# lab-emi/CleanUMamba

Measured on AMD Instinct MI355X. Metric: audio samples/sec/node (train step, E8, 10s@16kHz), higher is better.
Workload: dtype f16

## Files before the change

cleanumamba_amd/csrc/fft_lds.h:

```cpp
#pragma once
#include "common.h"

namespace cum {

__device__ __forceinline__ float2 cmul(float2 a, float2 b) { return make_float2(a.x * b.x - a.y * b.y, a.x * b.y + a.y * b.x); }
__device__ __forceinline__ float2 conjf2(float2 a) { return make_float2(a.x, -a.y); }
__device__ __forceinline__ float2 packed_bin(float2 za, float2 zb, float2 w) {
  const float2 c1 = make_float2(0.5f * (1.f + w.y), -0.5f * w.x), c2 = make_float2(0.5f * (1.f - w.y), 0.5f * w.x);
  const float2 p = cmul(c1, za), q = cmul(c2, conjf2(zb));
  return make_float2(p.x + q.x, p.y + q.y);
}
__device__ __forceinline__ double2 cmul(double2 a, double2 b) { return make_double2(a.x * b.x - a.y * b.y, a.x * b.y + a.y * b.x); }
__device__ __forceinline__ double2 packed_bin(double2 za, double2 zb, double2 w) {
  const double2 c1 = make_double2(0.5 * (1.0 + w.y), -0.5 * w.x), c2 = make_double2(0.5 * (1.0 - w.y), 0.5 * w.x);
  const double2 p = cmul(c1, za), q = cmul(c2, make_double2(zb.x, -zb.y));
  return make_double2(p.x + q.x, p.y + q.y);
}

template <typename T>
struct FftVec;
template <>
struct FftVec<float> {
  typedef float4 v4;
  typedef float2 v2;
  __device__ static __forceinline__ float4 mk4(float a, float b, float c, float d) { return make_float4(a, b, c, d); }
  __device__ static __forceinline__ float2 mk2(float a, float b) { return make_float2(a, b); }
};
template <>
struct FftVec<double> {
  typedef double4 v4;
  typedef double2 v2;
  __device__ static __forceinline__ double4 mk4(double a, double b, double c, double d) { return make_double4(a, b, c, d); }
  __device__ static __forceinline__ double2 mk2(double a, double b) { return make_double2(a, b); }
};

template <int H, typename T = float>
struct FusedFft {
  typedef typename FftVec<T>::v4 V4;
  typedef typename FftVec<T>::v2 V2;
  __device__ static __forceinline__ V4 mk4(T a, T b, T c, T d) { return FftVec<T>::mk4(a, b, c, d); }
  __device__ static __forceinline__ V2 mk2(T a, T b) { return FftVec<T>::mk2(a, b); }
  static constexpr int LOGH = H == 256 ? 8 : H == 512 ? 9 : 10;
  static constexpr bool LEAD2 = (LOGH & 1) != 0;
  static constexpr int PER = H / 64;
  static constexpr int SLOTS = H + H / 16;
  static constexpr int UNR = H == 1024 ? 2 : 1;

  __device__ static __forceinline__ int pad(int e) { return e + (e >> 4); }

  __device__ static __forceinline__ int pos(int k) {
    int p = 0, rem = k, L = H;
    if constexpr (LEAD2) {
      p = (rem & 1) * (H / 2);
      rem >>= 1;
      L = H / 2;
    }
#pragma unroll
    for (int s = 0; s < (LOGH / 2); ++s) {
      p += (rem & 3) * (L >> 2);
      rem >>= 2;
      L >>= 2;
    }
    return p;
  }

  __device__ static __forceinline__ V2 twiddle(const V2 *tw, int e, int L) {
    int m = e * (2 * H / L);
    const bool neg = m > H;
    m = neg ? m - H : m;
    V2 w = tw[m];
    if (neg) { w.x = -w.x; w.y = -w.y; }
    return w;
  }

  __device__ static __forceinline__ V4 cmul4(V4 v, V2 w) {
    return mk4(v.x * w.x - v.y * w.y, v.x * w.y + v.y * w.x, v.z * w.x - v.w * w.y, v.z * w.y + v.w * w.x);
  }
  __device__ static __forceinline__ V4 add4(V4 a, V4 b) { return mk4(a.x + b.x, a.y + b.y, a.z + b.z, a.w + b.w); }
  __device__ static __forceinline__ V4 sub4(V4 a, V4 b) { return mk4(a.x - b.x, a.y - b.y, a.z - b.z, a.w - b.w); }

  __device__ static __forceinline__ void stage_fence() {
    __builtin_amdgcn_fence(__ATOMIC_RELEASE, "wavefront");
    __builtin_amdgcn_wave_barrier();
    __builtin_amdgcn_fence(__ATOMIC_ACQUIRE, "wavefront");
  }

  __device__ static __forceinline__ void forward(V4 *buf, const V2 *tw, int lane) {
    int L = H;
    if constexpr (LEAD2) {
#pragma unroll UNR
      for (int i = 0; i < H / 128; ++i) {
        const int j = lane + 64 * i;
        const V4 a = buf[pad(j)], b = buf[pad(j + H / 2)];
        buf[pad(j)] = add4(a, b);
        buf[pad(j + H / 2)] = cmul4(sub4(a, b), twiddle(tw, j, H));
      }
      L = H / 2;
      stage_fence();
    }
#pragma unroll
    for (int st = 0; st < LOGH / 2; ++st, L >>= 2) {
      const int q4 = L >> 2;
#pragma unroll UNR
      for (int i = 0; i < H / 256; ++i) {
        const int q = lane + 64 * i;
        const int j = q & (q4 - 1), p = ((q - j) << 2) + j;
        const V4 a = buf[pad(p)], b = buf[pad(p + q4)], c = buf[pad(p + 2 * q4)], d = buf[pad(p + 3 * q4)];
        const V4 t0 = add4(a, c), t1 = sub4(a, c), t2 = add4(b, d), u = sub4(b, d);
        const V4 t3 = mk4(u.y, -u.x, u.w, -u.z);
        buf[pad(p)] = add4(t0, t2);
        if (L > 4) {
          buf[pad(p + q4)] = cmul4(add4(t1, t3), twiddle(tw, j, L));
          buf[pad(p + 2 * q4)] = cmul4(sub4(t0, t2), twiddle(tw, 2 * j, L));
          buf[pad(p + 3 * q4)] = cmul4(sub4(t1, t3), twiddle(tw, 3 * j, L));
        } else {
          buf[pad(p + q4)] = add4(t1, t3);
          buf[pad(p + 2 * q4)] = sub4(t0, t2);
          buf[pad(p + 3 * q4)] = sub4(t1, t3);
        }
      }
      stage_fence();
    }
  }

  __device__ static __forceinline__ void inverse_xy(V4 *buf, const V2 *tw, int lane) {
    auto ld = [&](int e) { const V4 v = buf[pad(e)]; return mk2(v.x, v.y); };
    auto st2 = [&](int e, float2 v) { float2 *q = reinterpret_cast<float2 *>(&buf[pad(e)]); *q = v; };
    auto cmulc = [](float2 v, float2 w) { return make_float2(v.x * w.x + v.y * w.y, v.y * w.x - v.x * w.y); };
    int L = 4;
#pragma unroll
    for (int stg = 0; stg < LOGH / 2; ++stg, L <<= 2) {
      const int q4 = L >> 2;
#pragma unroll UNR
      for (int i = 0; i < H / 256; ++i) {
        const int q = lane + 64 * i;
        const int j = q & (q4 - 1), p = ((q - j) << 2) + j;
        float2 a = ld(p), b = ld(p + q4), c = ld(p + 2 * q4), d = ld(p + 3 * q4);
        if (L > 4) {
          b = cmulc(b, twiddle(tw, j, L));
          c = cmulc(c, twiddle(tw, 2 * j, L));
          d = cmulc(d, twiddle(tw, 3 * j, L));
        }
        const float2 s0 = make_float2(a.x + c.x, a.y + c.y), s1 = make_float2(a.x - c.x, a.y - c.y);
        const float2 s2 = make_float2(b.x + d.x, b.y + d.y), u = make_float2(b.x - d.x, b.y - d.y);
        const float2 s3 = make_float2(-u.y, u.x);
        st2(p, make_float2(s0.x + s2.x, s0.y + s2.y));
        st2(p + q4, make_float2(s1.x + s3.x, s1.y + s3.y));
        st2(p + 2 * q4, make_float2(s0.x - s2.x, s0.y - s2.y));
        st2(p + 3 * q4, make_float2(s1.x - s3.x, s1.y - s3.y));
      }
      stage_fence();
    }
    if constexpr (LEAD2) {
#pragma unroll UNR
      for (int i = 0; i < H / 128; ++i) {
        const int j = lane + 64 * i;
        const float2 a = ld(j), b = cmulc(ld(j + H / 2), twiddle(tw, j, H));
        st2(j, make_float2(a.x + b.x, a.y + b.y));
        st2(j + H / 2, make_float2(a.x - b.x, a.y - b.y));
      }
      stage_fence();
    }
  }
};

}
```

cleanumamba_amd/csrc/stft_loss.hip:

```cpp
#include "common.h"
#include "fft_lds.h"

namespace cum {

constexpr int kLossRows = 8;
constexpr float kClamp = 1e-7f;

__device__ __forceinline__ int64_t reflect_index(int64_t s, int64_t len) {
  if (s < 0) s = -s;
  if (s >= len) s = 2 * (len - 1) - s;
  return s;
}

__global__ __launch_bounds__(256) void stft_frames_kernel(const float *__restrict__ x, int64_t len, int64_t x_sb,
                                                          int n_fft, int hop, int win_len,
                                                          const float *__restrict__ window,
                                                          float *__restrict__ frames, int64_t n_frames) {
  const int64_t f = blockIdx.x, b = blockIdx.y;
  const int off = (n_fft - win_len) / 2;
  const float *xb = x + b * x_sb;
  float *dst = frames + (b * n_frames + f) * n_fft;
  const int64_t s0 = f * hop - n_fft / 2;
  for (int n4 = threadIdx.x * 4; n4 < n_fft; n4 += 256 * 4) {
    float v[4];
// ... 112 lines not shown
          dm *= inv_mx * ((k == 0 || k == bins - 1) ? 1.f : 0.5f);
          out = make_float2(dm * vx.x, dm * vx.y);
        }
      }
      z[base + k] = out;
    }
  }
}

__global__ __launch_bounds__(256) void stft_loss_partials_packed_kernel(const float2 *__restrict__ zx,
                                                                        const float2 *__restrict__ zy, int64_t rows,
                                                                        int64_t n_frames, int H, int64_t frame0,
                                                                        const float2 *__restrict__ tw,
                                                                        float *__restrict__ partials) {
  __shared__ float red[4];
  const int64_t r0 = (int64_t)blockIdx.x * kLossRows;
  const int nrow = (int)min((int64_t)kLossRows, rows - r0);
  float s1 = 0.f, s2 = 0.f, s3 = 0.f;
  for (int r = 0; r < nrow; ++r) {
    if ((r0 + r) % n_frames < frame0) continue;
    const int64_t base = (r0 + r) * H;
    for (int k = threadIdx.x; k <= H; k += 256) {
      const int a = k == H ? 0 : k, b = k == 0 ? 0 : H - k;
      const float2 w = tw[k];
      const LossTerms t = loss_terms(packed_bin(zx[base + a], zx[base + b], w), packed_bin(zy[base + a], zy[base + b], w));
      const float d = t.my - t.mx;
      s1 += d * d;
      s2 += t.my * t.my;
      s3 += fabsf(logf(t.my) - logf(t.mx));
    }
  }
  s1 = block_sum_256(s1, red);
  s2 = block_sum_256(s2, red);
  s3 = block_sum_256(s3, red);
  if (threadIdx.x == 0) {
    partials[3 * (int64_t)blockIdx.x + 0] = s1;
    partials[3 * (int64_t)blockIdx.x + 1] = s2;
    partials[3 * (int64_t)blockIdx.x + 2] = s3;
  }
}

__device__ __forceinline__ float2 bin_grad(float2 vx, float2 vy, float c_sc, float c_mag) {
  const LossTerms t = loss_terms(vx, vy);
  if (!t.live) return make_float2(0.f, 0.f);
  const float inv_mx = 1.f / t.mx;
  const float lg = logf(t.mx) - logf(t.my);
  const float sgn = lg > 0.f ? 1.f : (lg < 0.f ? -1.f : 0.f);
  const float dm = (c_sc * (t.mx - t.my) + c_mag * sgn * inv_mx) * inv_mx;
  return make_float2(dm * vx.x, dm * vx.y);
}

__global__ __launch_bounds__(256) void stft_loss_grad_packed_kernel(const float2 *__restrict__ zx,
                                                                    const float2 *__restrict__ zy, int64_t rows,
                                                                    int64_t n_frames, int H, int64_t frame0,
                                                                    const float *__restrict__ stats,
                                                                    const float *__restrict__ g_sc,
                                                                    const float *__restrict__ g_mag, float inv_count,
                                                                    const float2 *__restrict__ tw,
                                                                    float2 *__restrict__ gz) {
  const int64_t r0 = (int64_t)blockIdx.x * kLossRows;
  const int nrow = (int)min((int64_t)kLossRows, rows - r0);
  const float c_sc = g_sc[0] / (stats[2] * stats[3]);
  const float c_mag = g_mag[0] * inv_count;
  for (int r = 0; r < nrow; ++r) {
    const bool in_band = (r0 + r) % n_frames >= frame0;
    const int64_t base = (r0 + r) * H;
    for (int j = threadIdx.x; j <= H / 2; j += 256) {
      const int m = j == 0 ? 0 : H - j;
      float2 oj = make_float2(0.f, 0.f), om = oj;
      if (in_band) {
        const float2 xj = zx[base + j], xm = zx[base + m], yj = zy[base + j], ym = zy[base + m];
        if (j == 0) {
          const float2 g0 = bin_grad(make_float2(xj.x + xj.y, 0.f), make_float2(yj.x + yj.y, 0.f), c_sc, c_mag);
          const float2 gh = bin_grad(make_float2(xj.x - xj.y, 0.f), make_float2(yj.x - yj.y, 0.f), c_sc, c_mag);
          oj = make_float2(g0.x + gh.x, g0.x - gh.x);
        } else {
          const float2 wj = tw[j], wm = tw[H - j];
          const float2 gj = bin_grad(packed_bin(xj, xm, wj), packed_bin(yj, ym, wj), c_sc, c_mag);
          const float2 gm = bin_grad(packed_bin(xm, xj, wm), packed_bin(ym, yj, wm), c_sc, c_mag);
          const float2 c1j = make_float2(0.5f * (1.f + wj.y), 0.5f * wj.x), c2j = make_float2(0.5f * (1.f - wj.y), 0.5f * wj.x);
          const float2 c1m = make_float2(0.5f * (1.f + wm.y), 0.5f * wm.x), c2m = make_float2(0.5f * (1.f - wm.y), 0.5f * wm.x);
          const float2 a = cmul(c1j, gj), b = cmul(c2m, conjf2(gm));
          oj = make_float2(a.x + b.x, a.y + b.y);
          const float2 c = cmul(c1m, gm), d = cmul(c2j, conjf2(gj));
          om = make_float2(c.x + d.x, c.y + d.y);
        }
      }
      gz[base + j] = oj;
      if (m != j) gz[base + m] = om;
    }
  }
}

__global__ __launch_bounds__(256) void stft_fold_kernel(const float *__restrict__ dframes, int64_t len, int n_fft,
                                                        int hop, int win_len, const float *__restrict__ window,
                                                        int64_t n_frames, float *__restrict__ dx, int64_t dx_sb,
                                                        int accumulate) {
  const int64_t m = (int64_t)blockIdx.x * 256 + threadIdx.x, b = blockIdx.y;
  if (m >= len) return;
  const int off = (n_fft - win_len) / 2, half = n_fft / 2;
  const float *src = dframes + b * n_frames * n_fft;
  float acc = 0.f;
  int64_t pos[3];
  int npos = 0;
  pos[npos++] = m + half;
  if (m >= 1 && m <= half) pos[npos++] = half - m;
  if (m <= len - 2 && m >= len - 1 - half) pos[npos++] = half + 2 * (len - 1) - m;
  for (int i = 0; i < npos; ++i) {
    const int64_t p = pos[i];
    if (p - off < 0) continue;
    int64_t f_hi = (p - off) / hop;
    if (f_hi > n_frames - 1) f_hi = n_frames - 1;
    int64_t f_lo = p - off - win_len + 1;
    f_lo = f_lo <= 0 ? 0 : (f_lo + hop - 1) / hop;
    for (int64_t f = f_lo; f <= f_hi; ++f) {
      const int n = (int)(p - f * hop);
      acc += window[n - off] * src[f * n_fft + n];
    }
  }
  float *o = dx + b * dx_sb + m;
  *o = accumulate ? *o + acc : acc;
}


__device__ __forceinline__ void fused_terms(float2 sx, float2 sy, float &s1, float &s2, float &s3) {
  const float px = fmaxf(sx.x * sx.x + sx.y * sx.y, kClamp), py = fmaxf(sy.x * sy.x + sy.y * sy.y, kClamp);
  const float d = __builtin_amdgcn_sqrtf(py) - __builtin_amdgcn_sqrtf(px);
  s1 = fmaf(d, d, s1);
  s2 += py;
  s3 += (0.5f * kLn2) * fabsf(__builtin_amdgcn_logf(py) - __builtin_amdgcn_logf(px));
}

__device__ __forceinline__ float2 fused_bin_grad(float2 vx, float2 vy, float c_sc, float c_mag) {
  const float pxr = vx.x * vx.x + vx.y * vx.y;
  if (!(pxr >= kClamp)) return make_float2(0.f, 0.f);
  const float py = fmaxf(vy.x * vy.x + vy.y * vy.y, kClamp);
  const float inv_mx = __builtin_amdgcn_rsqf(pxr);
  const float mx = pxr * inv_mx, my = __builtin_amdgcn_sqrtf(py);
  const float sgn = pxr > py ? 1.f : (pxr < py ? -1.f : 0.f);
  const float dm = (c_sc * (mx - my) + c_mag * sgn * inv_mx) * inv_mx;
  return make_float2(dm * vx.x, dm * vx.y);
}

struct FusedStftParams {
  const float *x, *y, *window, *tw;
  int64_t len, x_sb, y_sb, n_frames, frame0, n_total;
  int hop, win_len;
  float *partials;
  const float *stats, *g_sc, *g_mag;
  float inv_count;
  float *dframes;
};

template <int H>
__device__ __forceinline__ void fused_load_frame(const FusedStftParams &p, int64_t b, int64_t f, int lane, float4 *buf) {
  typedef FusedFft<H> F;
  const int n_fft = 2 * H, off = (n_fft - p.win_len) / 2;
  const float *xb = p.x + b * p.x_sb, *yb = p.y + b * p.y_sb;
  const int64_t s0 = f * p.hop - H;
  const bool inner = s0 >= 0 && s0 + n_fft <= p.len && ((off | p.win_len) & 1) == 0 &&
                     ((((uintptr_t)(xb + s0)) | ((uintptr_t)(yb + s0)) | ((uintptr_t)p.window)) & 7) == 0;
#pragma unroll 2
  for (int i = 0; i < F::PER; ++i) {
    const int m = lane + 64 * i, n = 2 * m;
    float4 z = make_float4(0.f, 0.f, 0.f, 0.f);
    if (n + 1 >= off && n < off + p.win_len) {
      float x0, x1, y0, y1, w0, w1;
      if (inner) {
        const float2 xv = *reinterpret_cast<const float2 *>(xb + s0 + n), yv = *reinterpret_cast<const float2 *>(yb + s0 + n);
        const float2 wv = *reinterpret_cast<const float2 *>(p.window + (n - off));
        x0 = xv.x; x1 = xv.y; y0 = yv.x; y1 = yv.y; w0 = wv.x; w1 = wv.y;
      } else {
        const int64_t i0 = reflect_index(s0 + n, p.len), i1 = reflect_index(s0 + n + 1, p.len);
        x0 = xb[i0]; x1 = xb[i1]; y0 = yb[i0]; y1 = yb[i1];
        const int wi = n - off;
        w0 = (wi >= 0 && wi < p.win_len) ? p.window[wi] : 0.f;
        w1 = (wi + 1 >= 0 && wi + 1 < p.win_len) ? p.window[wi + 1] : 0.f;
      }
      z = make_float4(w0 * x0, w1 * x1, w0 * y0, w1 * y1);
    }
    buf[F::pad(m)] = z;
  }
}

template <int H>
__device__ __forceinline__ void fused_load_tables(const FusedStftParams &p, float2 *tw) {
  for (int k = threadIdx.x; k <= H; k += blockDim.x) tw[k] = reinterpret_cast<const float2 *>(p.tw)[k];
  __syncthreads();
}

constexpr int kFusedWaves = 4;

template <int H>
__global__ __launch_bounds__(64 * kFusedWaves) __attribute__((amdgpu_waves_per_eu(H == 256 ? 6 : (H == 512 ? 4 : 2)))) void stft_fused_fwd_kernel(const FusedStftParams p) {
  typedef FusedFft<H> F;
  __shared__ __attribute__((aligned(16))) float4 s_buf[kFusedWaves][F::SLOTS];
  __shared__ float2 s_tw[H + 1];
  __shared__ float s_red[3][kFusedWaves];
  const int lane = threadIdx.x & 63, wave = uniform(threadIdx.x >> 6);
  fused_load_tables<H>(p, s_tw);
  float4 *buf = s_buf[wave];
  float s1 = 0.f, s2 = 0.f, s3 = 0.f;
  const int nw = gridDim.x * kFusedWaves, n_total = (int)p.n_total, n_frames = (int)p.n_frames;
  for (int fr = blockIdx.x * kFusedWaves + wave; fr < n_total; fr += nw) {
    const int b = fr / n_frames, f = fr - b * n_frames;
    if (f < p.frame0) continue;
    fused_load_frame<H>(p, b, f, lane, buf);
    F::stage_fence();
    F::forward(buf, s_tw, lane);
#pragma unroll 1
    for (int i = 0; i <= F::PER / 2; ++i) {
      const int j = lane + 64 * i;
      if (j > H / 2) break;
      const int m = j == 0 ? 0 : H - j;
      const float4 vj = buf[F::pad(F::pos(j))], vm = buf[F::pad(F::pos(m))];
      const float2 xj = make_float2(vj.x, vj.y), yj = make_float2(vj.z, vj.w), xm = make_float2(vm.x, vm.y), ym = make_float2(vm.z, vm.w);
      if (j == 0) {
        fused_terms(make_float2(xj.x + xj.y, 0.f), make_float2(yj.x + yj.y, 0.f), s1, s2, s3);
        fused_terms(make_float2(xj.x - xj.y, 0.f), make_float2(yj.x - yj.y, 0.f), s1, s2, s3);
      } else {
        const float2 wj = s_tw[j];
        fused_terms(packed_bin(xj, xm, wj), packed_bin(yj, ym, wj), s1, s2, s3);
        if (m != j) {
          const float2 wm = s_tw[m];
          fused_terms(packed_bin(xm, xj, wm), packed_bin(ym, yj, wm), s1, s2, s3);
        }
      }
    }
    F::stage_fence();
  }
  float v[3] = {s1, s2, s3};
#pragma unroll
  for (int j = 0; j < 3; ++j) {
#pragma unroll
    for (int o = 32; o >= 1; o >>= 1) v[j] += __shfl_xor(v[j], o, 64);
    if (lane == 0) s_red[j][wave] = v[j];
  }
  __syncthreads();
  if (threadIdx.x < 3) {
    float t = 0.f;
#pragma unroll
    for (int w = 0; w < kFusedWaves; ++w) t += s_red[threadIdx.x][w];
    p.partials[3 * (int64_t)blockIdx.x + threadIdx.x] = t;
  }
}

template <int H>
__global__ __launch_bounds__(64 * kFusedWaves) __attribute__((amdgpu_waves_per_eu(H == 256 ? 6 : (H == 512 ? 4 : 2)))) void stft_fused_bwd_kernel(const FusedStftParams p) {
  typedef FusedFft<H> F;
  __shared__ __attribute__((aligned(16))) float4 s_buf[kFusedWaves][F::SLOTS];
  __shared__ float2 s_tw[H + 1];
  const int lane = threadIdx.x & 63, wave = uniform(threadIdx.x >> 6);
  fused_load_tables<H>(p, s_tw);
  float4 *buf = s_buf[wave];
  const float c_sc = p.g_sc[0] / (p.stats[2] * p.stats[3]);
  const float c_mag = p.g_mag[0] * p.inv_count;
  const int n_fft = 2 * H, off = (n_fft - p.win_len) / 2;
  const int nw = gridDim.x * kFusedWaves, n_total = (int)p.n_total, n_frames = (int)p.n_frames;
  for (int fr = blockIdx.x * kFusedWaves + wave; fr < n_total; fr += nw) {
    const int b = fr / n_frames, f = fr - b * n_frames;
    float *dst = p.dframes + (int64_t)fr * n_fft;
    if (f < p.frame0) {
#pragma unroll
      for (int i = 0; i < F::PER; ++i) {
        const int n = 2 * (lane + 64 * i);
        if (n + 1 >= off && n < off + p.win_len) *reinterpret_cast<float2 *>(dst + n) = make_float2(0.f, 0.f);
      }
      continue;
    }
    fused_load_frame<H>(p, b, f, lane, buf);
    F::stage_fence();
    F::forward(buf, s_tw, lane);
#pragma unroll 1
    for (int i = 0; i <= F::PER / 2; ++i) {
      const int j = lane + 64 * i;
      if (j > H / 2) break;
      const int m = j == 0 ? 0 : H - j;
      const int pj = F::pad(F::pos(j)), pm = F::pad(F::pos(m));
      const float4 vj = buf[pj], vm = buf[pm];
      const float2 xj = make_float2(vj.x, vj.y), yj = make_float2(vj.z, vj.w), xm = make_float2(vm.x, vm.y), ym = make_float2(vm.z, vm.w);
      float2 oj, om = make_float2(0.f, 0.f);
      if (j == 0) {
        const float2 g0 = fused_bin_grad(make_float2(xj.x + xj.y, 0.f), make_float2(yj.x + yj.y, 0.f), c_sc, c_mag);
        const float2 gh = fused_bin_grad(make_float2(xj.x - xj.y, 0.f), make_float2(yj.x - yj.y, 0.f), c_sc, c_mag);
        oj = make_float2(g0.x + gh.x, g0.x - gh.x);
      } else {
        const float2 wj = s_tw[j], wm = s_tw[H - j];
        const float2 gj = fused_bin_grad(packed_bin(xj, xm, wj), packed_bin(yj, ym, wj), c_sc, c_mag);
        const float2 gm = fused_bin_grad(packed_bin(xm, xj, wm), packed_bin(ym, yj, wm), c_sc, c_mag);
        const float2 c1j = make_float2(0.5f * (1.f + wj.y), 0.5f * wj.x), c2j = make_float2(0.5f * (1.f - wj.y), 0.5f * wj.x);
        const float2 c1m = make_float2(0.5f * (1.f + wm.y), 0.5f * wm.x), c2m = make_float2(0.5f * (1.f - wm.y), 0.5f * wm.x);
        const float2 a = cmul(c1j, gj), bq = cmul(c2m, conjf2(gm));
        oj = make_float2(a.x + bq.x, a.y + bq.y);
        const float2 c = cmul(c1m, gm), d = cmul(c2j, conjf2(gj));
        om = make_float2(c.x + d.x, c.y + d.y);
      }
      *reinterpret_cast<float2 *>(&buf[pj]) = oj;
      if (m != j) *reinterpret_cast<float2 *>(&buf[pm]) = om;
    }
    F::stage_fence();
    F::inverse_xy(buf, s_tw, lane);
#pragma unroll
    for (int i = 0; i < F::PER; ++i) {
      const int mm = lane + 64 * i, n = 2 * mm;
      if (n + 1 >= off && n < off + p.win_len) {
        const float4 v = buf[F::pad(mm)];
        *reinterpret_cast<float2 *>(dst + n) = make_float2(v.x, v.y);
      }
    }
    F::stage_fence();
  }
}

}

using namespace cum;

static int check_resolution(int64_t len, int n_fft, int hop, int win_len, int64_t n_frames) {
  CUM_REQUIRE(n_fft >= 8 && n_fft % 4 == 0 && hop > 0 && win_len > 0 && win_len <= n_fft, "stft: bad resolution");
  CUM_REQUIRE(len > n_fft / 2, "stft: signal shorter than the reflect padding");
  CUM_REQUIRE(n_frames == 1 + len / hop, "stft: n_frames must be 1 + len / hop");
  return CUM_OK;
}

extern "C" int cum_stft_frames(const float *x, int64_t batch, int64_t len, int64_t x_stride_b, int32_t n_fft,
                               int32_t hop, int32_t win_length, const float *window, float *frames, int64_t n_frames,
                               void *stream) {
  CUM_REQUIRE(batch >= 0 && batch < 65536, "stft_frames: bad batch");
  if (int rc = check_resolution(len, n_fft, hop, win_length, n_frames)) return rc;
  if (batch == 0) return CUM_OK;
  CUM_REQUIRE(x && window && frames, "stft_frames: null pointer");
  hipLaunchKernelGGL(stft_frames_kernel, dim3((unsigned)n_frames, (unsigned)batch), dim3(256), 0, (hipStream_t)stream,
                     x, len, x_stride_b, n_fft, hop, win_length, window, frames, n_frames);
  CUM_CHECK_LAUNCH();
  return CUM_OK;
}

extern "C" int64_t cum_stft_loss_workspace_elems(int64_t batch, int64_t n_frames) {
  return 3 * cdiv64(batch * n_frames, kLossRows);
}

extern "C" int cum_stft_loss_fwd(const float *spec_x, const float *spec_y, int64_t batch, int64_t n_frames,
                                 int32_t bins, int64_t frame0, float *workspace, float *stats, void *stream) {
  CUM_REQUIRE(batch > 0 && n_frames > 0 && bins > 0 && frame0 >= 0 && frame0 < n_frames, "stft_loss_fwd: bad shape");
  CUM_REQUIRE(spec_x && spec_y && workspace && stats, "stft_loss_fwd: null pointer");
  const int64_t rows = batch * n_frames, parts = cdiv64(rows, kLossRows);
  hipLaunchKernelGGL(stft_loss_partials_kernel, dim3((unsigned)parts), dim3(256), 0, (hipStream_t)stream,
                     (const float2 *)spec_x, (const float2 *)spec_y, rows, n_frames, bins, frame0, workspace);
  const double count = (double)batch * (double)(n_frames - frame0) * (double)bins;
  hipLaunchKernelGGL(stft_loss_finalize_kernel, dim3(1), dim3(1024), 0, (hipStream_t)stream, workspace, parts, count,
                     stats);
  CUM_CHECK_LAUNCH();
  return CUM_OK;
}

extern "C" int cum_stft_loss_bwd(const float *spec_x, const float *spec_y, int64_t batch, int64_t n_frames,
                                 int32_t bins, int64_t frame0, const float *stats, const float *g_sc,
                                 const float *g_mag, float *zspec, void *stream) {
  CUM_REQUIRE(batch > 0 && n_frames > 0 && bins > 0 && frame0 >= 0 && frame0 < n_frames, "stft_loss_bwd: bad shape");
  CUM_REQUIRE(spec_x && spec_y && stats && g_sc && g_mag && zspec, "stft_loss_bwd: null pointer");
  const int64_t rows = batch * n_frames, parts = cdiv64(rows, kLossRows);
  const double count = (double)batch * (double)(n_frames - frame0) * (double)bins;
  hipLaunchKernelGGL(stft_loss_grad_kernel, dim3((unsigned)parts), dim3(256), 0, (hipStream_t)stream,
                     (const float2 *)spec_x, (const float2 *)spec_y, rows, n_frames, bins, frame0, stats, g_sc, g_mag,
                     (float)(1.0 / count), (float2 *)zspec);
  CUM_CHECK_LAUNCH();
  return CUM_OK;
}

extern "C" int cum_stft_fold(const float *dframes, int64_t batch, int64_t len, int32_t n_fft, int32_t hop,
                             int32_t win_length, const float *window, int64_t n_frames, float *dx,
                             int64_t dx_stride_b, int32_t accumulate, void *stream) {
  CUM_REQUIRE(batch >= 0 && batch < 65536, "stft_fold: bad batch");
  if (int rc = check_resolution(len, n_fft, hop, win_length, n_frames)) return rc;
  if (batch == 0) return CUM_OK;
  CUM_REQUIRE(dframes && window && dx, "stft_fold: null pointer");
  hipLaunchKernelGGL(stft_fold_kernel, dim3((unsigned)cdiv64(len, 256), (unsigned)batch), dim3(256), 0,
                     (hipStream_t)stream, dframes, len, n_fft, hop, win_length, window, n_frames, dx, dx_stride_b,
                     accumulate);
  CUM_CHECK_LAUNCH();
  return CUM_OK;
}

extern "C" int cum_stft_loss_fwd_packed(const float *zx, const float *zy, int64_t batch, int64_t n_frames, int32_t n_fft,
                                        int64_t frame0, const float *twiddle, float *workspace, float *stats,
                                        void *stream) {
  CUM_REQUIRE(batch > 0 && n_frames > 0 && n_fft >= 8 && n_fft % 4 == 0 && frame0 >= 0 && frame0 < n_frames,
              "stft_loss_fwd_packed: bad shape");
  CUM_REQUIRE(zx && zy && twiddle && workspace && stats, "stft_loss_fwd_packed: null pointer");
  const int64_t rows = batch * n_frames, parts = cdiv64(rows, kLossRows);
  const int H = n_fft / 2;
  hipLaunchKernelGGL(stft_loss_partials_packed_kernel, dim3((unsigned)parts), dim3(256), 0, (hipStream_t)stream,
                     (const float2 *)zx, (const float2 *)zy, rows, n_frames, H, frame0, (const float2 *)twiddle,
                     workspace);
  const double count = (double)batch * (double)(n_frames - frame0) * (double)(H + 1);
  hipLaunchKernelGGL(stft_loss_finalize_kernel, dim3(1), dim3(1024), 0, (hipStream_t)stream, workspace, parts, count,
                     stats);
  CUM_CHECK_LAUNCH();
  return CUM_OK;
}

extern "C" int cum_stft_loss_bwd_packed(const float *zx, const float *zy, int64_t batch, int64_t n_frames, int32_t n_fft,
                                        int64_t frame0, const float *stats, const float *g_sc, const float *g_mag,
                                        const float *twiddle, float *gz, void *stream) {
  CUM_REQUIRE(batch > 0 && n_frames > 0 && n_fft >= 8 && n_fft % 4 == 0 && frame0 >= 0 && frame0 < n_frames,
              "stft_loss_bwd_packed: bad shape");
  CUM_REQUIRE(zx && zy && stats && g_sc && g_mag && twiddle && gz, "stft_loss_bwd_packed: null pointer");
  const int64_t rows = batch * n_frames, parts = cdiv64(rows, kLossRows);
  const int H = n_fft / 2;
  const double count = (double)batch * (double)(n_frames - frame0) * (double)(H + 1);
  hipLaunchKernelGGL(stft_loss_grad_packed_kernel, dim3((unsigned)parts), dim3(256), 0, (hipStream_t)stream,
                     (const float2 *)zx, (const float2 *)zy, rows, n_frames, H, frame0, stats, g_sc, g_mag,
                     (float)(1.0 / count), (const float2 *)twiddle, (float2 *)gz);
  CUM_CHECK_LAUNCH();
  return CUM_OK;
}

extern "C" int cum_stft_fused_supported(int32_t n_fft) { return n_fft == 512 || n_fft == 1024 || n_fft == 2048; }

static int fused_grid(int64_t n_total) {
  const int64_t want = cdiv64(n_total, 4 * kFusedWaves);
  const int64_t g = want < 256 ? (want < 1 ? 1 : want) : (want < 2048 ? cdiv64(want, 256) * 256 : 2048);
  return (int)g;
}

extern "C" int64_t cum_stft_fused_workspace_elems(int64_t batch, int64_t n_frames) { return 3 * (int64_t)fused_grid(batch * n_frames); }

static int fused_params(FusedStftParams &p, const float *x, const float *y, int64_t batch, int64_t len, int64_t x_sb,
                        int64_t y_sb, int32_t n_fft, int32_t hop, int32_t win_length, const float *window,
                        const float *twiddle, int64_t n_frames, int64_t frame0) {
  CUM_REQUIRE(cum_stft_fused_supported(n_fft), "stft_fused: n_fft must be 512, 1024 or 2048");
  CUM_REQUIRE(batch > 0 && batch < 65536 && frame0 >= 0 && frame0 < n_frames && batch * n_frames < 2147483647LL,
              "stft_fused: bad batch / frame0");
  if (int rc = check_resolution(len, n_fft, hop, win_length, n_frames)) return rc;
  CUM_REQUIRE(x && y && window && twiddle, "stft_fused: null pointer");
  p.x = x; p.y = y; p.window = window; p.tw = twiddle;
  p.len = len; p.x_sb = x_sb; p.y_sb = y_sb; p.n_frames = n_frames; p.frame0 = frame0; p.n_total = batch * n_frames;
  p.hop = hop; p.win_len = win_length;
  return CUM_OK;
}

extern "C" int cum_stft_fused_fwd(const float *x, const float *y, int64_t batch, int64_t len, int64_t x_stride_b,
                                  int64_t y_stride_b, int32_t n_fft, int32_t hop, int32_t win_length, const float *window,
                                  const float *twiddle, int64_t n_frames, int64_t frame0, float *workspace, float *stats,
                                  void *stream) {
  FusedStftParams p{};
  if (int rc = fused_params(p, x, y, batch, len, x_stride_b, y_stride_b, n_fft, hop, win_length, window, twiddle, n_frames, frame0)) return rc;
  CUM_REQUIRE(workspace && stats, "stft_fused_fwd: null pointer");
  p.partials = workspace;
  const int grid = fused_grid(p.n_total);
  hipStream_t st = (hipStream_t)stream;
  if (n_fft == 512) hipLaunchKernelGGL(stft_fused_fwd_kernel<256>, dim3(grid), dim3(64 * kFusedWaves), 0, st, p);
  else if (n_fft == 1024) hipLaunchKernelGGL(stft_fused_fwd_kernel<512>, dim3(grid), dim3(64 * kFusedWaves), 0, st, p);
  else hipLaunchKernelGGL(stft_fused_fwd_kernel<1024>, dim3(grid), dim3(64 * kFusedWaves), 0, st, p);
  CUM_CHECK_LAUNCH();
  const double count = (double)batch * (double)(n_frames - frame0) * (double)(n_fft / 2 + 1);
  hipLaunchKernelGGL(stft_loss_finalize_kernel, dim3(1), dim3(1024), 0, st, workspace, (int64_t)grid, count, stats);
  CUM_CHECK_LAUNCH();
  return CUM_OK;
}
// ... 20 lines not shown
```

Before: 130.4 million.

## Use register-resident radix-16 pass FFT for 1024-point fused STFT loss

Adds a specialised 1024-point FFT for the fused STFT loss forward and backward kernels. It keeps 16 points per lane in registers and performs two radix-16 passes (pairs of radix-4 stages) with LDS transposes between them, replacing the five LDS round-trip stages of the generic in-place FFT. The final radix-4 stage is merged into the bin-pair gradient and terms computation. Frames are loaded straight into registers on the interior path. The cost is higher register pressure and a new custom LDS slot layout that needs careful index mapping and may reduce occupancy.

```diff
diff --git a/cleanumamba_amd/csrc/fft_lds.h b/cleanumamba_amd/csrc/fft_lds.h
--- a/cleanumamba_amd/csrc/fft_lds.h
+++ b/cleanumamba_amd/csrc/fft_lds.h
@@ -164,4 +164,112 @@
   }
 };
 
+struct PassFft1024 {
+  typedef FusedFft<1024, float> F;
+  static constexpr int H = 1024, SLOTS = 64 * 17 + 4;
+
+  __device__ static __forceinline__ void lane_br(int lane, int &b, int &r) {
+    b = (lane & 3) | ((lane >> 1) & 12);
+    r = ((lane >> 5) << 1) | (__builtin_popcount((lane >> 2) & 7) & 1);
+  }
+  __device__ static __forceinline__ int slot_t(int hi, int lo) { return 17 * lo + hi; }
+  __device__ static __forceinline__ int slot_c(int d, int g) { return d * 260 + (g & 0xF0) + ((g >> 2) & 3) + 4 * (g & 3); }
+  __device__ static __forceinline__ int klow(int b, int k) { return (b >> 2) + 4 * (b & 3) + 16 * (k >> 2) + 64 * (k & 3); }
+  __device__ static __forceinline__ void groups(int lane, int it, int &g, int &gm) {
+    int b, r;
+    lane_br(lane, b, r);
+    g = (b >> 2) + 4 * (b & 3) + 16 * r + 64 * it;
+    gm = g == 0 ? 128 : 256 - g;
+  }
+
+  __device__ static __forceinline__ void dif4(float4 &a, float4 &b, float4 &c, float4 &d) {
+    const float4 t0 = F::add4(a, c), t1 = F::sub4(a, c), t2 = F::add4(b, d), u = F::sub4(b, d);
+    const float4 t3 = make_float4(u.y, -u.x, u.w, -u.z);
+    a = F::add4(t0, t2); b = F::add4(t1, t3); c = F::sub4(t0, t2); d = F::sub4(t1, t3);
+  }
+  __device__ static __forceinline__ void dit4(float2 &a, float2 &b, float2 &c, float2 &d) {
+    const float2 s0 = make_float2(a.x + c.x, a.y + c.y), s1 = make_float2(a.x - c.x, a.y - c.y);
+    const float2 s2 = make_float2(b.x + d.x, b.y + d.y), u = make_float2(b.x - d.x, b.y - d.y);
+    const float2 s3 = make_float2(-u.y, u.x);
+    a = make_float2(s0.x + s2.x, s0.y + s2.y); b = make_float2(s1.x + s3.x, s1.y + s3.y);
+    c = make_float2(s0.x - s2.x, s0.y - s2.y); d = make_float2(s1.x - s3.x, s1.y - s3.y);
+  }
+  __device__ static __forceinline__ float2 cmulc(float2 v, float2 w) { return make_float2(v.x * w.x + v.y * w.y, v.y * w.x - v.x * w.y); }
+
+  template <int L1, int L2, int JS>
+  __device__ static __forceinline__ void dif_pair(float4 (&v)[16], const float2 *tw, int j0) {
+#pragma unroll
+    for (int q = 0; q < 4; ++q) {
+      dif4(v[q], v[q + 4], v[q + 8], v[q + 12]);
+      const int j = j0 + JS * q;
+      v[q + 4] = F::cmul4(v[q + 4], F::twiddle(tw, j, L1));
+      v[q + 8] = F::cmul4(v[q + 8], F::twiddle(tw, 2 * j, L1));
+      v[q + 12] = F::cmul4(v[q + 12], F::twiddle(tw, 3 * j, L1));
+    }
+    const float2 w1 = F::twiddle(tw, j0, L2), w2 = F::twiddle(tw, 2 * j0, L2), w3 = F::twiddle(tw, 3 * j0, L2);
+#pragma unroll
+    for (int q = 0; q < 4; ++q) {
+      dif4(v[4 * q], v[4 * q + 1], v[4 * q + 2], v[4 * q + 3]);
+      v[4 * q + 1] = F::cmul4(v[4 * q + 1], w1);
+      v[4 * q + 2] = F::cmul4(v[4 * q + 2], w2);
+      v[4 * q + 3] = F::cmul4(v[4 * q + 3], w3);
+    }
+  }
+  template <int L1, int L2, int JS>
+  __device__ static __forceinline__ void dit_pair(float2 (&v)[16], const float2 *tw, int j0) {
+    const float2 w1 = F::twiddle(tw, j0, L2), w2 = F::twiddle(tw, 2 * j0, L2), w3 = F::twiddle(tw, 3 * j0, L2);
+#pragma unroll
+    for (int q = 0; q < 4; ++q) {
+      v[4 * q + 1] = cmulc(v[4 * q + 1], w1);
+      v[4 * q + 2] = cmulc(v[4 * q + 2], w2);
+      v[4 * q + 3] = cmulc(v[4 * q + 3], w3);
+      dit4(v[4 * q], v[4 * q + 1], v[4 * q + 2], v[4 * q + 3]);
+    }
+#pragma unroll
+    for (int q = 0; q < 4; ++q) {
+      const int j = j0 + JS * q;
+      v[q + 4] = cmulc(v[q + 4], F::twiddle(tw, j, L1));
+      v[q + 8] = cmulc(v[q + 8], F::twiddle(tw, 2 * j, L1));
+      v[q + 12] = cmulc(v[q + 12], F::twiddle(tw, 3 * j, L1));
+      dit4(v[q], v[q + 4], v[q + 8], v[q + 12]);
+    }
+  }
+
+  __device__ static __forceinline__ void forward(float4 (&v)[16], float4 *buf, const float2 *tw, int lane) {
+    asm volatile("" : "+v"(lane));
+    dif_pair<1024, 256, 64>(v, tw, lane);
+#pragma unroll
+    for (int i = 0; i < 16; ++i) buf[slot_t(i, lane)] = v[i];
+    F::stage_fence();
+    int b, r;
+    lane_br(lane, b, r);
+#pragma unroll
+    for (int k = 0; k < 16; ++k) v[k] = buf[slot_t(b, r + 4 * k)];
+    F::stage_fence();
+    dif_pair<64, 16, 4>(v, tw, r);
+#pragma unroll
+    for (int k = 0; k < 16; ++k) buf[slot_c(r, klow(b, k))] = v[k];
+    F::stage_fence();
+  }
+
+  __device__ static __forceinline__ void inverse_xy(float2 (&v)[16], float4 *buf, const float2 *tw, int lane) {
+    auto ld = [&](int s) { const float2 *q = reinterpret_cast<const float2 *>(&buf[s]); return *q; };
+    auto st2 = [&](int s, float2 x) { float2 *q = reinterpret_cast<float2 *>(&buf[s]); *q = x; };
+    asm volatile("" : "+v"(lane));
+    int b, r;
+    lane_br(lane, b, r);
+#pragma unroll
+    for (int k = 0; k < 16; ++k) v[k] = ld(slot_c(r, klow(b, k)));
+    F::stage_fence();
+    dit_pair<64, 16, 4>(v, tw, r);
+#pragma unroll
+    for (int k = 0; k < 16; ++k) st2(slot_t(b, r + 4 * k), v[k]);
+    F::stage_fence();
+#pragma unroll
+    for (int i = 0; i < 16; ++i) v[i] = ld(slot_t(i, lane));
+    F::stage_fence();
+    dit_pair<1024, 256, 64>(v, tw, lane);
+  }
+};
+
 }
diff --git a/cleanumamba_amd/csrc/stft_loss.hip b/cleanumamba_amd/csrc/stft_loss.hip
--- a/cleanumamba_amd/csrc/stft_loss.hip
+++ b/cleanumamba_amd/csrc/stft_loss.hip
@@ -288,35 +288,102 @@
   float *dframes;
 };
 
+struct FusedFrameSrc {
+  const float *xb, *yb;
+  int64_t s0;
+  int off;
+  bool inner;
+};
+
+template <int H>
+__device__ __forceinline__ FusedFrameSrc fused_frame_src(const FusedStftParams &p, int64_t b, int64_t f) {
+  const int n_fft = 2 * H;
+  FusedFrameSrc s;
+  s.off = (n_fft - p.win_len) / 2;
+  s.xb = p.x + b * p.x_sb;
+  s.yb = p.y + b * p.y_sb;
+  s.s0 = f * p.hop - H;
+  s.inner = s.s0 >= 0 && s.s0 + n_fft <= p.len && ((s.off | p.win_len) & 1) == 0 &&
+            ((((uintptr_t)(s.xb + s.s0)) | ((uintptr_t)(s.yb + s.s0)) | ((uintptr_t)p.window)) & 7) == 0;
+  return s;
+}
+
+__device__ __forceinline__ float4 fused_load_point(const FusedStftParams &p, const FusedFrameSrc &s, int m) {
+  const int n = 2 * m;
+  float4 z = make_float4(0.f, 0.f, 0.f, 0.f);
+  if (n + 1 >= s.off && n < s.off + p.win_len) {
+    float x0, x1, y0, y1, w0, w1;
+    if (s.inner) {
+      const float2 xv = *reinterpret_cast<const float2 *>(s.xb + s.s0 + n), yv = *reinterpret_cast<const float2 *>(s.yb + s.s0 + n);
+      const float2 wv = *reinterpret_cast<const float2 *>(p.window + (n - s.off));
+      x0 = xv.x; x1 = xv.y; y0 = yv.x; y1 = yv.y; w0 = wv.x; w1 = wv.y;
+    } else {
+      const int64_t i0 = reflect_index(s.s0 + n, p.len), i1 = reflect_index(s.s0 + n + 1, p.len);
+      x0 = s.xb[i0]; x1 = s.xb[i1]; y0 = s.yb[i0]; y1 = s.yb[i1];
+      const int wi = n - s.off;
+      w0 = (wi >= 0 && wi < p.win_len) ? p.window[wi] : 0.f;
+      w1 = (wi + 1 >= 0 && wi + 1 < p.win_len) ? p.window[wi + 1] : 0.f;
+    }
+    z = make_float4(w0 * x0, w1 * x1, w0 * y0, w1 * y1);
+  }
+  return z;
+}
+
 template <int H>
 __device__ __forceinline__ void fused_load_frame(const FusedStftParams &p, int64_t b, int64_t f, int lane, float4 *buf) {
   typedef FusedFft<H> F;
-  const int n_fft = 2 * H, off = (n_fft - p.win_len) / 2;
-  const float *xb = p.x + b * p.x_sb, *yb = p.y + b * p.y_sb;
-  const int64_t s0 = f * p.hop - H;
-  const bool inner = s0 >= 0 && s0 + n_fft <= p.len && ((off | p.win_len) & 1) == 0 &&
-                     ((((uintptr_t)(xb + s0)) | ((uintptr_t)(yb + s0)) | ((uintptr_t)p.window)) & 7) == 0;
+  const FusedFrameSrc s = fused_frame_src<H>(p, b, f);
 #pragma unroll 2
   for (int i = 0; i < F::PER; ++i) {
-    const int m = lane + 64 * i, n = 2 * m;
-    float4 z = make_float4(0.f, 0.f, 0.f, 0.f);
-    if (n + 1 >= off && n < off + p.win_len) {
-      float x0, x1, y0, y1, w0, w1;
-      if (inner) {
-        const float2 xv = *reinterpret_cast<const float2 *>(xb + s0 + n), yv = *reinterpret_cast<const float2 *>(yb + s0 + n);
-        const float2 wv = *reinterpret_cast<const float2 *>(p.window + (n - off));
-        x0 = xv.x; x1 = xv.y; y0 = yv.x; y1 = yv.y; w0 = wv.x; w1 = wv.y;
-      } else {
-        const int64_t i0 = reflect_index(s0 + n, p.len), i1 = reflect_index(s0 + n + 1, p.len);
-        x0 = xb[i0]; x1 = xb[i1]; y0 = yb[i0]; y1 = yb[i1];
-        const int wi = n - off;
-        w0 = (wi >= 0 && wi < p.win_len) ? p.window[wi] : 0.f;
-        w1 = (wi + 1 >= 0 && wi + 1 < p.win_len) ? p.window[wi + 1] : 0.f;
-      }
-      z = make_float4(w0 * x0, w1 * x1, w0 * y0, w1 * y1);
-    }
-    buf[F::pad(m)] = z;
-  }
+    const int m = lane + 64 * i;
+    buf[F::pad(m)] = fused_load_point(p, s, m);
+  }
+}
+
+__device__ __forceinline__ void fused_load_frame_regs(const FusedStftParams &p, int64_t b, int64_t f, int lane, float4 *buf,
+                                                      float4 (&v)[16]) {
+  const FusedFrameSrc s = fused_frame_src<1024>(p, b, f);
+  if (s.inner) {
+    const float *xs = s.xb + s.s0, *ys = s.yb + s.s0, *ws = p.window - s.off;
+    float2 xv[16], yv[16], wv[16];
+#pragma unroll
+    for (int i = 0; i < 16; ++i) {
+      const int n = 2 * (lane + 64 * i);
+      xv[i] = yv[i] = wv[i] = make_float2(0.f, 0.f);
+      if (n >= s.off && n < s.off + p.win_len) {
+        xv[i] = *reinterpret_cast<const float2 *>(xs + n);
+        yv[i] = *reinterpret_cast<const float2 *>(ys + n);
+        wv[i] = *reinterpret_cast<const float2 *>(ws + n);
+      }
+    }
+#pragma unroll
+    for (int i = 0; i < 16; ++i) v[i] = make_float4(wv[i].x * xv[i].x, wv[i].y * xv[i].y, wv[i].x * yv[i].x, wv[i].y * yv[i].y);
+  } else {
+#pragma unroll 1
+    for (int i = 0; i < 16; ++i) buf[lane + 64 * i] = fused_load_point(p, s, lane + 64 * i);
+#pragma unroll
+    for (int i = 0; i < 16; ++i) v[i] = buf[lane + 64 * i];
+    FusedFft<1024>::stage_fence();
+  }
+}
+
+__device__ __forceinline__ void fused_pair_grad(float4 vj, float4 vm, float2 wj, float2 wm, float c_sc, float c_mag,
+                                                float2 &oj, float2 &om) {
+  const float2 xj = make_float2(vj.x, vj.y), yj = make_float2(vj.z, vj.w), xm = make_float2(vm.x, vm.y), ym = make_float2(vm.z, vm.w);
+  const float2 gj = fused_bin_grad(packed_bin(xj, xm, wj), packed_bin(yj, ym, wj), c_sc, c_mag);
+  const float2 gm = fused_bin_grad(packed_bin(xm, xj, wm), packed_bin(ym, yj, wm), c_sc, c_mag);
+  const float2 c1j = make_float2(0.5f * (1.f + wj.y), 0.5f * wj.x), c2j = make_float2(0.5f * (1.f - wj.y), 0.5f * wj.x);
+  const float2 c1m = make_float2(0.5f * (1.f + wm.y), 0.5f * wm.x), c2m = make_float2(0.5f * (1.f - wm.y), 0.5f * wm.x);
+  const float2 a = cmul(c1j, gj), bq = cmul(c2m, conjf2(gm));
+  oj = make_float2(a.x + bq.x, a.y + bq.y);
+  const float2 c = cmul(c1m, gm), d = cmul(c2j, conjf2(gj));
+  om = make_float2(c.x + d.x, c.y + d.y);
+}
+
+__device__ __forceinline__ void fused_pair_terms(float4 vj, float4 vm, float2 wj, float2 wm, float &s1, float &s2, float &s3) {
+  const float2 xj = make_float2(vj.x, vj.y), yj = make_float2(vj.z, vj.w), xm = make_float2(vm.x, vm.y), ym = make_float2(vm.z, vm.w);
+  fused_terms(packed_bin(xj, xm, wj), packed_bin(yj, ym, wj), s1, s2, s3);
+  fused_terms(packed_bin(xm, xj, wm), packed_bin(ym, yj, wm), s1, s2, s3);
 }
 
 template <int H>
@@ -330,7 +397,7 @@
 template <int H>
 __global__ __launch_bounds__(64 * kFusedWaves) __attribute__((amdgpu_waves_per_eu(H == 256 ? 6 : (H == 512 ? 4 : 2)))) void stft_fused_fwd_kernel(const FusedStftParams p) {
   typedef FusedFft<H> F;
-  __shared__ __attribute__((aligned(16))) float4 s_buf[kFusedWaves][F::SLOTS];
+  __shared__ __attribute__((aligned(16))) float4 s_buf[kFusedWaves][H == 1024 ? PassFft1024::SLOTS : F::SLOTS];
   __shared__ float2 s_tw[H + 1];
   __shared__ float s_red[3][kFusedWaves];
   const int lane = threadIdx.x & 63, wave = uniform(threadIdx.x >> 6);
@@ -341,25 +408,59 @@
   for (int fr = blockIdx.x * kFusedWaves + wave; fr < n_total; fr += nw) {
     const int b = fr / n_frames, f = fr - b * n_frames;
     if (f < p.frame0) continue;
-    fused_load_frame<H>(p, b, f, lane, buf);
-    F::stage_fence();
-    F::forward(buf, s_tw, lane);
+    if constexpr (H == 1024) {
+      typedef PassFft1024 P;
+      float4 v[16];
+      fused_load_frame_regs(p, b, f, lane, buf, v);
+      P::forward(v, buf, s_tw, lane);
 #pragma unroll 1
-    for (int i = 0; i <= F::PER / 2; ++i) {
-      const int j = lane + 64 * i;
-      if (j > H / 2) break;
-      const int m = j == 0 ? 0 : H - j;
-      const float4 vj = buf[F::pad(F::pos(j))], vm = buf[F::pad(F::pos(m))];
-      const float2 xj = make_float2(vj.x, vj.y), yj = make_float2(vj.z, vj.w), xm = make_float2(vm.x, vm.y), ym = make_float2(vm.z, vm.w);
-      if (j == 0) {
-        fused_terms(make_float2(xj.x + xj.y, 0.f), make_float2(yj.x + yj.y, 0.f), s1, s2, s3);
-        fused_terms(make_float2(xj.x - xj.y, 0.f), make_float2(yj.x - yj.y, 0.f), s1, s2, s3);
-      } else {
-        const float2 wj = s_tw[j];
-        fused_terms(packed_bin(xj, xm, wj), packed_bin(yj, ym, wj), s1, s2, s3);
-        if (m != j) {
-          const float2 wm = s_tw[m];
-          fused_terms(packed_bin(xm, xj, wm), packed_bin(ym, yj, wm), s1, s2, s3);
+      for (int it = 0; it < 2; ++it) {
+        int g, gm;
+        P::groups(lane, it, g, gm);
+        float4 za[4], zb[4];
+#pragma unroll
+        for (int d = 0; d < 4; ++d) { za[d] = buf[P::slot_c(d, g)]; zb[d] = buf[P::slot_c(d, gm)]; }
+        P::dif4(za[0], za[1], za[2], za[3]);
+        P::dif4(zb[0], zb[1], zb[2], zb[3]);
+        if (it == 0 && g == 0) {
+          const float4 z0 = za[0], zh = za[2];
+          fused_terms(make_float2(z0.x + z0.y, 0.f), make_float2(z0.z + z0.w, 0.f), s1, s2, s3);
+          fused_terms(make_float2(z0.x - z0.y, 0.f), make_float2(z0.z - z0.w, 0.f), s1, s2, s3);
+          const float2 wh = s_tw[512];
+          fused_terms(packed_bin(make_float2(zh.x, zh.y), make_float2(zh.x, zh.y), wh),
+                      packed_bin(make_float2(zh.z, zh.w), make_float2(zh.z, zh.w), wh), s1, s2, s3);
+          fused_pair_terms(za[1], za[3], s_tw[256], s_tw[768], s1, s2, s3);
+          fused_pair_terms(zb[0], zb[3], s_tw[128], s_tw[896], s1, s2, s3);
+          fused_pair_terms(zb[1], zb[2], s_tw[384], s_tw[640], s1, s2, s3);
+        } else {
+#pragma unroll
+          for (int d = 0; d < 4; ++d) {
+            const int j = g + 256 * d;
+            fused_pair_terms(za[d], zb[3 - d], s_tw[j], s_tw[H - j], s1, s2, s3);
+          }
+        }
+      }
+    } else {
+      fused_load_frame<H>(p, b, f, lane, buf);
+      F::stage_fence();
+      F::forward(buf, s_tw, lane);
+#pragma unroll 1
+      for (int i = 0; i <= F::PER / 2; ++i) {
+        const int j = lane + 64 * i;
+        if (j > H / 2) break;
+        const int m = j == 0 ? 0 : H - j;
+        const float4 vj = buf[F::pad(F::pos(j))], vm = buf[F::pad(F::pos(m))];
+        const float2 xj = make_float2(vj.x, vj.y), yj = make_float2(vj.z, vj.w), xm = make_float2(vm.x, vm.y), ym = make_float2(vm.z, vm.w);
+        if (j == 0) {
+          fused_terms(make_float2(xj.x + xj.y, 0.f), make_float2(yj.x + yj.y, 0.f), s1, s2, s3);
+          fused_terms(make_float2(xj.x - xj.y, 0.f), make_float2(yj.x - yj.y, 0.f), s1, s2, s3);
+        } else {
+          const float2 wj = s_tw[j];
+          fused_terms(packed_bin(xj, xm, wj), packed_bin(yj, ym, wj), s1, s2, s3);
+          if (m != j) {
+            const float2 wm = s_tw[m];
+            fused_terms(packed_bin(xm, xj, wm), packed_bin(ym, yj, wm), s1, s2, s3);
+          }
         }
       }
     }
@@ -384,7 +485,7 @@
 template <int H>
 __global__ __launch_bounds__(64 * kFusedWaves) __attribute__((amdgpu_waves_per_eu(H == 256 ? 6 : (H == 512 ? 4 : 2)))) void stft_fused_bwd_kernel(const FusedStftParams p) {
   typedef FusedFft<H> F;
-  __shared__ __attribute__((aligned(16))) float4 s_buf[kFusedWaves][F::SLOTS];
+  __shared__ __attribute__((aligned(16))) float4 s_buf[kFusedWaves][H == 1024 ? PassFft1024::SLOTS : F::SLOTS];
   __shared__ float2 s_tw[H + 1];
   const int lane = threadIdx.x & 63, wave = uniform(threadIdx.x >> 6);
   fused_load_tables<H>(p, s_tw);
@@ -404,44 +505,96 @@
       }
       continue;
     }
-    fused_load_frame<H>(p, b, f, lane, buf);
-    F::stage_fence();
-    F::forward(buf, s_tw, lane);
+    if constexpr (H == 1024) {
+      typedef PassFft1024 P;
+      {
+        float4 v[16];
+        fused_load_frame_regs(p, b, f, lane, buf, v);
+        P::forward(v, buf, s_tw, lane);
+      }
 #pragma unroll 1
-    for (int i = 0; i <= F::PER / 2; ++i) {
-      const int j = lane + 64 * i;
-      if (j > H / 2) break;
-      const int m = j == 0 ? 0 : H - j;
-      const int pj = F::pad(F::pos(j)), pm = F::pad(F::pos(m));
-      const float4 vj = buf[pj], vm = buf[pm];
-      const float2 xj = make_float2(vj.x, vj.y), yj = make_float2(vj.z, vj.w), xm = make_float2(vm.x, vm.y), ym = make_float2(vm.z, vm.w);
-      float2 oj, om = make_float2(0.f, 0.f);
-      if (j == 0) {
-        const float2 g0 = fused_bin_grad(make_float2(xj.x + xj.y, 0.f), make_float2(yj.x + yj.y, 0.f), c_sc, c_mag);
-        const float2 gh = fused_bin_grad(make_float2(xj.x - xj.y, 0.f), make_float2(yj.x - yj.y, 0.f), c_sc, c_mag);
-        oj = make_float2(g0.x + gh.x, g0.x - gh.x);
-      } else {
-        const float2 wj = s_tw[j], wm = s_tw[H - j];
-        const float2 gj = fused_bin_grad(packed_bin(xj, xm, wj), packed_bin(yj, ym, wj), c_sc, c_mag);
-        const float2 gm = fused_bin_grad(packed_bin(xm, xj, wm), packed_bin(ym, yj, wm), c_sc, c_mag);
-        const float2 c1j = make_float2(0.5f * (1.f + wj.y), 0.5f * wj.x), c2j = make_float2(0.5f * (1.f - wj.y), 0.5f * wj.x);
-        const float2 c1m = make_float2(0.5f * (1.f + wm.y), 0.5f * wm.x), c2m = make_float2(0.5f * (1.f - wm.y), 0.5f * wm.x);
-        const float2 a = cmul(c1j, gj), bq = cmul(c2m, conjf2(gm));
-        oj = make_float2(a.x + bq.x, a.y + bq.y);
-        const float2 c = cmul(c1m, gm), d = cmul(c2j, conjf2(gj));
-        om = make_float2(c.x + d.x, c.y + d.y);
-      }
-      *reinterpret_cast<float2 *>(&buf[pj]) = oj;
-      if (m != j) *reinterpret_cast<float2 *>(&buf[pm]) = om;
-    }
-    F::stage_fence();
-    F::inverse_xy(buf, s_tw, lane);
-#pragma unroll
-    for (int i = 0; i < F::PER; ++i) {
-      const int mm = lane + 64 * i, n = 2 * mm;
-      if (n + 1 >= off && n < off + p.win_len) {
-        const float4 v = buf[F::pad(mm)];
-        *reinterpret_cast<float2 *>(dst + n) = make_float2(v.x, v.y);
+      for (int it = 0; it < 2; ++it) {
+        int g, gm;
+        P::groups(lane, it, g, gm);
+        float4 za[4], zb[4];
+#pragma unroll
+        for (int d = 0; d < 4; ++d) { za[d] = buf[P::slot_c(d, g)]; zb[d] = buf[P::slot_c(d, gm)]; }
+        P::dif4(za[0], za[1], za[2], za[3]);
+        P::dif4(zb[0], zb[1], zb[2], zb[3]);
+        float2 ga[4], gb[4];
+        if (it == 0 && g == 0) {
+          const float4 z0 = za[0];
+          const float2 g0 = fused_bin_grad(make_float2(z0.x + z0.y, 0.f), make_float2(z0.z + z0.w, 0.f), c_sc, c_mag);
+          const float2 gh = fused_bin_grad(make_float2(z0.x - z0.y, 0.f), make_float2(z0.z - z0.w, 0.f), c_sc, c_mag);
+          ga[0] = make_float2(g0.x + gh.x, g0.x - gh.x);
+          float2 unused;
+          fused_pair_grad(za[2], za[2], s_tw[512], s_tw[512], c_sc, c_mag, ga[2], unused);
+          fused_pair_grad(za[1], za[3], s_tw[256], s_tw[768], c_sc, c_mag, ga[1], ga[3]);
+          fused_pair_grad(zb[0], zb[3], s_tw[128], s_tw[896], c_sc, c_mag, gb[0], gb[3]);
+          fused_pair_grad(zb[1], zb[2], s_tw[384], s_tw[640], c_sc, c_mag, gb[1], gb[2]);
+        } else {
+#pragma unroll
+          for (int d = 0; d < 4; ++d) {
+            const int j = g + 256 * d;
+            fused_pair_grad(za[d], zb[3 - d], s_tw[j], s_tw[H - j], c_sc, c_mag, ga[d], gb[3 - d]);
+          }
+        }
+        P::dit4(ga[0], ga[1], ga[2], ga[3]);
+        P::dit4(gb[0], gb[1], gb[2], gb[3]);
+#pragma unroll
+        for (int d = 0; d < 4; ++d) {
+          *reinterpret_cast<float2 *>(&buf[P::slot_c(d, g)]) = ga[d];
+          *reinterpret_cast<float2 *>(&buf[P::slot_c(d, gm)]) = gb[d];
+        }
+      }
+      F::stage_fence();
+      float2 w[16];
+      P::inverse_xy(w, buf, s_tw, lane);
+#pragma unroll
+      for (int i = 0; i < 16; ++i) {
+        const int n = 2 * (lane + 64 * i);
+        if (n + 1 >= off && n < off + p.win_len) *reinterpret_cast<float2 *>(dst + n) = w[i];
+      }
+    } else {
+      fused_load_frame<H>(p, b, f, lane, buf);
+      F::stage_fence();
+      F::forward(buf, s_tw, lane);
+#pragma unroll 1
+      for (int i = 0; i <= F::PER / 2; ++i) {
+        const int j = lane + 64 * i;
+        if (j > H / 2) break;
+        const int m = j == 0 ? 0 : H - j;
+        const int pj = F::pad(F::pos(j)), pm = F::pad(F::pos(m));
+        const float4 vj = buf[pj], vm = buf[pm];
+        const float2 xj = make_float2(vj.x, vj.y), yj = make_float2(vj.z, vj.w), xm = make_float2(vm.x, vm.y), ym = make_float2(vm.z, vm.w);
+        float2 oj, om = make_float2(0.f, 0.f);
+        if (j == 0) {
+          const float2 g0 = fused_bin_grad(make_float2(xj.x + xj.y, 0.f), make_float2(yj.x + yj.y, 0.f), c_sc, c_mag);
+          const float2 gh = fused_bin_grad(make_float2(xj.x - xj.y, 0.f), make_float2(yj.x - yj.y, 0.f), c_sc, c_mag);
+          oj = make_float2(g0.x + gh.x, g0.x - gh.x);
+        } else {
+          const float2 wj = s_tw[j], wm = s_tw[H - j];
+          const float2 gj = fused_bin_grad(packed_bin(xj, xm, wj), packed_bin(yj, ym, wj), c_sc, c_mag);
+          const float2 gm = fused_bin_grad(packed_bin(xm, xj, wm), packed_bin(ym, yj, wm), c_sc, c_mag);
+          const float2 c1j = make_float2(0.5f * (1.f + wj.y), 0.5f * wj.x), c2j = make_float2(0.5f * (1.f - wj.y), 0.5f * wj.x);
+          const float2 c1m = make_float2(0.5f * (1.f + wm.y), 0.5f * wm.x), c2m = make_float2(0.5f * (1.f - wm.y), 0.5f * wm.x);
+          const float2 a = cmul(c1j, gj), bq = cmul(c2m, conjf2(gm));
+          oj = make_float2(a.x + bq.x, a.y + bq.y);
+          const float2 c = cmul(c1m, gm), d = cmul(c2j, conjf2(gj));
+          om = make_float2(c.x + d.x, c.y + d.y);
+        }
+        *reinterpret_cast<float2 *>(&buf[pj]) = oj;
+        if (m != j) *reinterpret_cast<float2 *>(&buf[pm]) = om;
+      }
+      F::stage_fence();
+      F::inverse_xy(buf, s_tw, lane);
+#pragma unroll
+      for (int i = 0; i < F::PER; ++i) {
+        const int mm = lane + 64 * i, n = 2 * mm;
+        if (n + 1 >= off && n < off + p.win_len) {
+          const float4 v = buf[F::pad(mm)];
+          *reinterpret_cast<float2 *>(dst + n) = make_float2(v.x, v.y);
+        }
       }
     }
     F::stage_fence();
```

Result: no change. 131.1 million, median of 6 (+0.5%).
